# budzianowski/VAEB

Measured on AMD Instinct MI355X. Metric: SGVB training images/sec + ELBO at MNIST 784-500-20, batch 100, higher is better.
Workload: dtype f32; 1 GPU; MNIST 784-500-20 Bernoulli decoder, LB estimator, L=1, Adagrad lr 0.01; global_batch=100, batch_per_gpu=100, parallelism=dp1

## Files before the change

include/vaeb_diag.h:

```cpp
#ifndef VAEB_DIAG_H
#define VAEB_DIAG_H

#include "vaeb_hip.h"

#ifdef __cplusplus
extern "C" {
#endif

int vaeb_profile_steps(vaeb_ctx* ctx, int32_t n_steps, float* out_ms_per_kernel,
                       int32_t* out_kernel_ids, int32_t max_kernels, int32_t* out_n_kernels);
int vaeb_kernel_name(int32_t kernel_id, char* out, int32_t cap);

enum vaeb_graph_mode { VAEB_GRAPH_OFF = 0, VAEB_GRAPH_NOT_CAPTURED = 1, VAEB_GRAPH_REPLAY = 2,
                       VAEB_GRAPH_EAGER_FALLBACK = 3 };
int vaeb_graph_status(vaeb_ctx* ctx, int32_t* mode, char* msg, int32_t cap);
int vaeb_time_update_many(vaeb_ctx* ctx, const int32_t* batch_indices, int32_t n, float* out_gpu_ms,
                          double* out_enqueue_ms);
int vaeb_busy(vaeb_ctx* ctx, int32_t us);
int vaeb_comm_info(vaeb_ctx* ctx, int32_t* rccl_version, int32_t* dp_overlap, int32_t* world);
int vaeb_dp_plan(const vaeb_config* cfg, int32_t world, int32_t rank, int32_t sharded, int32_t bucket,
                 int64_t* out_P, int64_t* runs, int32_t* out_nrun, int64_t* own, int32_t* out_nown,
                 int32_t* out_book, int64_t* foreign, int32_t* out_nforeign);
int vaeb_dw2_plan(const vaeb_config* cfg, int32_t* out_width, int32_t* out_paired, int32_t* out_workers,
                  int32_t* out_free_cus, int32_t* out_split, int32_t* ranges, int32_t cap);
int vaeb_dp_rank_update(vaeb_ctx* ctx, int32_t world, int32_t rank, int32_t bucket, const float* grad_sum,
                        int64_t n_grad, const float* theta_gathered, int32_t finish);
int vaeb_get_shadow(vaeb_ctx* ctx, uint16_t* out, int64_t n);
int vaeb_debug_timeline(vaeb_ctx* ctx, int32_t batch_index, uint64_t* out, int64_t cap,
                        int32_t* out_launches);

int vaeb_test_gemm_bf16(vaeb_ctx* ctx, int32_t a_kouter, int32_t b_kouter, int32_t M, int32_t N, int32_t K,
                        const float* A, const float* B, float* C, int32_t ksplit);
int vaeb_bench_gemm_bf16(vaeb_ctx* ctx, int32_t a_kouter, int32_t b_kouter, int32_t M, int32_t N, int32_t K,
                         int32_t tile_n, int32_t reps, float* out_ms);

#ifdef __cplusplus
}
#endif
#endif
```

vaeb_amd/_lib.py:

```python
from __future__ import annotations

import ctypes
import os

import numpy as np

HERE = os.path.dirname(os.path.abspath(__file__))
LIB_PATH = os.path.join(HERE, "libvaeb_hip.so")
if os.environ.get("VAEB_LIB_VARIANT"):
    LIB_PATH = os.path.join(HERE, f"libvaeb_hip_{os.environ['VAEB_LIB_VARIANT']}.so")

DEC_BERNOULLI, DEC_GAUSSIAN = 0, 1
EST_LB, EST_LA, EST_FV, EST_FVS = 0, 1, 2, 3
OBJ_SUM_PRIOR, OBJ_MEAN_MAP = 0, 1
EPS_PHILOX, EPS_HOST = 0, 1
DTYPE_F32, DTYPE_BF16, DTYPE_F16 = 0, 1, 2

EXPORTS = [
    "vaeb_last_error", "vaeb_version", "vaeb_create", "vaeb_destroy", "vaeb_num_params",
    "vaeb_set_data", "vaeb_set_params", "vaeb_get_params", "vaeb_set_adagrad_state",
    "vaeb_get_adagrad_state", "vaeb_set_fv_state", "vaeb_get_fv_state", "vaeb_set_eps_mode",
    "vaeb_push_eps", "vaeb_set_step", "vaeb_get_step", "vaeb_update", "vaeb_update_async", "vaeb_update_many",
    "vaeb_epoch_elbo", "vaeb_synchronize", "vaeb_validate", "vaeb_reconstruct", "vaeb_reconstruct_sampled",
    "vaeb_reconstruct_full", "vaeb_decode", "vaeb_encode", "vaeb_marginal_ll", "vaeb_marginal_ll_resident",
    "vaeb_comm_unique_id", "vaeb_comm_init", "vaeb_comm_count", "vaeb_set_valid_data", "vaeb_validate_resident",
    "vaeb_checkpoint_save", "vaeb_checkpoint_load", "vaeb_get_grads", "vaeb_get_activation", "vaeb_push_fv_noise",
    "vaeb_ae_create", "vaeb_ae_destroy", "vaeb_ae_num_params", "vaeb_ae_set_data", "vaeb_ae_set_params",
    "vaeb_ae_get_params", "vaeb_ae_set_adagrad_state", "vaeb_ae_get_adagrad_state", "vaeb_ae_train",
    "vaeb_ae_train_many", "vaeb_ae_reconstruct", "vaeb_ae_encode", "vaeb_ae_decode",
]
DIAG_EXPORTS = ["vaeb_profile_steps", "vaeb_kernel_name", "vaeb_debug_timeline", "vaeb_test_gemm_bf16",
                "vaeb_bench_gemm_bf16", "vaeb_graph_status", "vaeb_comm_info", "vaeb_time_update_many", "vaeb_busy",
                "vaeb_dp_plan", "vaeb_dp_rank_update", "vaeb_get_shadow", "vaeb_dw2_plan"]
GRAPH_MODES = {0: "off", 1: "not_captured", 2: "replay", 3: "eager_fallback"}
AE_MAX_LAYERS = 8
AE_BINARY, AE_CONT = 0, 1
ACT = {"tanh": 0, "sigmoid": 1, "relu": 2}


class VaebConfig(ctypes.Structure):
    _fields_ = [
        ("D", ctypes.c_int32), ("H", ctypes.c_int32), ("Z", ctypes.c_int32), ("B", ctypes.c_int32),
        ("B_global", ctypes.c_int32), ("row_offset", ctypes.c_int32), ("L", ctypes.c_int32),
        ("decoder", ctypes.c_int32), ("estimator", ctypes.c_int32), ("objective", ctypes.c_int32),
        ("lr", ctypes.c_float), ("adagrad_eps", ctypes.c_float), ("device", ctypes.c_int32),
        ("max_eval_rows", ctypes.c_int32), ("use_graph", ctypes.c_int32), ("keep_grads", ctypes.c_int32),
        ("dtype", ctypes.c_int32), ("reserved", ctypes.c_int32 * 5),
    ]


class AEConfigC(ctypes.Structure):
    _fields_ = [
        ("Dobs", ctypes.c_int32), ("n_enc", ctypes.c_int32), ("Denc", ctypes.c_int32 * 8),
        ("Dz", ctypes.c_int32), ("n_dec", ctypes.c_int32), ("Ddec", ctypes.c_int32 * 8),
        ("otype", ctypes.c_int32), ("act", ctypes.c_int32), ("s2", ctypes.c_float), ("eta", ctypes.c_float),
        ("max_batch", ctypes.c_int32), ("device", ctypes.c_int32), ("reserved", ctypes.c_int32 * 4),
    ]


class VaebError(RuntimeError):
    pass


_lib = None

_F = ctypes.POINTER(ctypes.c_float)
_I64 = ctypes.c_int64
_P = ctypes.c_void_p


def load():
    global _lib
    if _lib is not None:
        return _lib
    if not os.path.exists(LIB_PATH):
        raise VaebError(f"{LIB_PATH} not found: build it with `python -c 'import __graft_entry__ as g; g.build()'`")
    if not os.environ.get("VAEB_LIB_VARIANT"):
        from ._buildinfo import check_stamp
        why = check_stamp(LIB_PATH)
        if why:
            raise VaebError(f"stale {LIB_PATH}: {why}; rebuild with `python -c 'import __graft_entry__ as g; g.build()'`")
    lib = ctypes.CDLL(LIB_PATH)
    sig = {
        "vaeb_last_error": ([], ctypes.c_char_p),
        "vaeb_version": ([ctypes.POINTER(ctypes.c_int32)] * 2, ctypes.c_int),
        "vaeb_create": ([ctypes.POINTER(VaebConfig), ctypes.POINTER(_P)], ctypes.c_int),
        "vaeb_destroy": ([_P], ctypes.c_int),
        "vaeb_num_params": ([_P, ctypes.POINTER(_I64)], ctypes.c_int),
        "vaeb_set_data": ([_P, _F, _I64], ctypes.c_int),
        "vaeb_set_params": ([_P, _F, _I64], ctypes.c_int),
        "vaeb_get_params": ([_P, _F, _I64], ctypes.c_int),
        "vaeb_set_adagrad_state": ([_P, _F, _I64], ctypes.c_int),
        "vaeb_get_adagrad_state": ([_P, _F, _I64], ctypes.c_int),
        "vaeb_set_fv_state": ([_P, _F, _F, _F, _F, _I64], ctypes.c_int),
        "vaeb_get_fv_state": ([_P, _F, _F, _F, _F, _I64], ctypes.c_int),
        "vaeb_set_eps_mode": ([_P, ctypes.c_int32, ctypes.c_uint64], ctypes.c_int),
        "vaeb_push_eps": ([_P, _F, _I64, ctypes.c_int32], ctypes.c_int),
        "vaeb_set_step": ([_P, _I64], ctypes.c_int),
        "vaeb_get_step": ([_P, ctypes.POINTER(_I64)], ctypes.c_int),
        "vaeb_comm_count": ([_P, ctypes.POINTER(ctypes.c_int32)], ctypes.c_int),
        "vaeb_set_valid_data": ([_P, _F, _I64], ctypes.c_int),
        "vaeb_validate_resident": ([_P, ctypes.POINTER(ctypes.c_double)], ctypes.c_int),
        "vaeb_checkpoint_save": ([_P, ctypes.c_char_p], ctypes.c_int),
        "vaeb_checkpoint_load": ([_P, ctypes.c_char_p], ctypes.c_int),
        "vaeb_update": ([_P, ctypes.c_int32, _F], ctypes.c_int),
        "vaeb_update_async": ([_P, ctypes.c_int32], ctypes.c_int),
        "vaeb_update_many": ([_P, ctypes.POINTER(ctypes.c_int32), ctypes.c_int32], ctypes.c_int),
        "vaeb_epoch_elbo": ([_P, ctypes.POINTER(ctypes.c_double), ctypes.POINTER(_I64)], ctypes.c_int),
        "vaeb_synchronize": ([_P], ctypes.c_int),
        "vaeb_validate": ([_P, _F, _I64, ctypes.POINTER(ctypes.c_double)], ctypes.c_int),
        "vaeb_reconstruct": ([_P, _F, _I64, _F], ctypes.c_int),
        "vaeb_reconstruct_sampled": ([_P, _F, _I64, ctypes.c_int32, _F], ctypes.c_int),
        "vaeb_reconstruct_full": ([_P, _F, _I64, ctypes.c_int32, _F, _F], ctypes.c_int),
        "vaeb_decode": ([_P, _F, _I64, _F, _F], ctypes.c_int),
        "vaeb_encode": ([_P, _F, _I64, _F, _F], ctypes.c_int),
        "vaeb_marginal_ll": ([_P, _F, _I64, ctypes.c_int32, ctypes.POINTER(ctypes.c_double), _F], ctypes.c_int),
        "vaeb_marginal_ll_resident": ([_P, ctypes.c_int32, ctypes.POINTER(ctypes.c_double)], ctypes.c_int),
        "vaeb_comm_unique_id": ([ctypes.POINTER(ctypes.c_uint8)], ctypes.c_int),
        "vaeb_comm_init": ([_P, ctypes.POINTER(ctypes.c_uint8), ctypes.c_int32, ctypes.c_int32], ctypes.c_int),
        "vaeb_get_grads": ([_P, _F, _I64], ctypes.c_int),
        "vaeb_get_activation": ([_P, ctypes.c_char_p, _F, _I64], ctypes.c_int),
        "vaeb_profile_steps": ([_P, ctypes.c_int32, _F, ctypes.POINTER(ctypes.c_int32), ctypes.c_int32,
                                ctypes.POINTER(ctypes.c_int32)], ctypes.c_int),
        "vaeb_kernel_name": ([ctypes.c_int32, ctypes.c_char_p, ctypes.c_int32], ctypes.c_int),
        "vaeb_graph_status": ([_P, ctypes.POINTER(ctypes.c_int32), ctypes.c_char_p, ctypes.c_int32], ctypes.c_int),
        "vaeb_comm_info": ([_P] + [ctypes.POINTER(ctypes.c_int32)] * 3, ctypes.c_int),
        "vaeb_busy": ([_P, ctypes.c_int32], ctypes.c_int),
        "vaeb_dp_plan": ([ctypes.POINTER(VaebConfig)] + [ctypes.c_int32] * 4 +
                         [ctypes.POINTER(_I64), ctypes.POINTER(_I64), ctypes.POINTER(ctypes.c_int32),
                          ctypes.POINTER(_I64), ctypes.POINTER(ctypes.c_int32), ctypes.POINTER(ctypes.c_int32),
                          ctypes.POINTER(_I64), ctypes.POINTER(ctypes.c_int32)], ctypes.c_int),
        "vaeb_dp_rank_update": ([_P] + [ctypes.c_int32] * 3 + [_F, _I64, _F, ctypes.c_int32], ctypes.c_int),
        "vaeb_dw2_plan": ([ctypes.POINTER(VaebConfig)] + [ctypes.POINTER(ctypes.c_int32)] * 6 + [ctypes.c_int32],
                          ctypes.c_int),
        "vaeb_get_shadow": ([_P, ctypes.POINTER(ctypes.c_uint16), _I64], ctypes.c_int),
        "vaeb_time_update_many": ([_P, ctypes.POINTER(ctypes.c_int32), ctypes.c_int32, _F,
                                   ctypes.POINTER(ctypes.c_double)], ctypes.c_int),
        "vaeb_debug_timeline": ([_P, ctypes.c_int32, ctypes.POINTER(ctypes.c_uint64), _I64,
                                 ctypes.POINTER(ctypes.c_int32)], ctypes.c_int),
        "vaeb_test_gemm_bf16": ([_P] + [ctypes.c_int32] * 5 + [_F, _F, _F, ctypes.c_int32], ctypes.c_int),
        "vaeb_bench_gemm_bf16": ([_P] + [ctypes.c_int32] * 7 + [_F], ctypes.c_int),
        "vaeb_push_fv_noise": ([_P, _F, _I64], ctypes.c_int),
        "vaeb_ae_create": ([ctypes.POINTER(AEConfigC), ctypes.POINTER(_P)], ctypes.c_int),
        "vaeb_ae_destroy": ([_P], ctypes.c_int),
        "vaeb_ae_num_params": ([_P, ctypes.POINTER(_I64)], ctypes.c_int),
        "vaeb_ae_set_data": ([_P, _F, _I64], ctypes.c_int),
        "vaeb_ae_set_params": ([_P, _F, _I64], ctypes.c_int),
        "vaeb_ae_get_params": ([_P, _F, _I64], ctypes.c_int),
        "vaeb_ae_set_adagrad_state": ([_P, _F, _I64], ctypes.c_int),
        "vaeb_ae_get_adagrad_state": ([_P, _F, _I64], ctypes.c_int),
        "vaeb_ae_train": ([_P, ctypes.POINTER(ctypes.c_int32), ctypes.c_int32, _F], ctypes.c_int),
        "vaeb_ae_train_many": ([_P, ctypes.POINTER(ctypes.c_int32), ctypes.c_int32, ctypes.c_int32, _F], ctypes.c_int),
        "vaeb_ae_reconstruct": ([_P, _F, _I64, _F], ctypes.c_int),
        "vaeb_ae_encode": ([_P, _F, _I64, _F], ctypes.c_int),
        "vaeb_ae_decode": ([_P, _F, _I64, _F], ctypes.c_int),
    }
    for name, (args, res) in sig.items():
        fn = getattr(lib, name)
        fn.argtypes = args
        fn.restype = res
    _lib = lib
    return lib


def check(rc):
    if rc != 0:
        msg = _lib.vaeb_last_error().decode(errors="replace") if _lib is not None else "?"
        raise VaebError(f"libvaeb_hip error {rc}: {msg}")


def dp_plan(D, H, Z, world, rank, bucket=2, sharded=True, decoder=DEC_BERNOULLI):
    lib = load()
    cfg = VaebConfig()
    cfg.D, cfg.H, cfg.Z, cfg.B, cfg.L = D, H, Z, 1, 1
    cfg.decoder = decoder
    P = _I64()
    runs = (_I64 * 9)()
    own = (_I64 * 12)()
    foreign = (_I64 * 12)()
    nrun, nown, book, nfor = (ctypes.c_int32() for _ in range(4))
    check(lib.vaeb_dp_plan(ctypes.byref(cfg), world, rank, int(bool(sharded)), bucket, ctypes.byref(P), runs,
                           ctypes.byref(nrun), own, ctypes.byref(nown), ctypes.byref(book), foreign,
                           ctypes.byref(nfor)))
    return {"P": P.value,
            "runs": [(runs[3 * j], runs[3 * j + 1], runs[3 * j + 2]) for j in range(nrun.value)],
            "own": [(own[2 * k], own[2 * k + 1]) for k in range(nown.value)],
            "book": bool(book.value),
            "foreign": [(foreign[2 * k], foreign[2 * k + 1]) for k in range(nfor.value)]}


def dw2_plan(D, H, Z, B, decoder=DEC_BERNOULLI):
    lib = load()
    cfg = VaebConfig()
    cfg.D, cfg.H, cfg.Z, cfg.B, cfg.B_global, cfg.L = D, H, Z, B, B, 1
    cfg.decoder = decoder
    width, paired, workers, free, split = (ctypes.c_int32() for _ in range(5))
    check(lib.vaeb_dw2_plan(ctypes.byref(cfg), ctypes.byref(width), ctypes.byref(paired), ctypes.byref(workers),
                            ctypes.byref(free), ctypes.byref(split), None, 0))
    r = (ctypes.c_int32 * (4 * workers.value))()
    check(lib.vaeb_dw2_plan(ctypes.byref(cfg), None, None, None, None, None, r, workers.value))
    return {"width": width.value, "paired": bool(paired.value), "workers": workers.value, "free_cus": free.value,
            "split": split.value, "ranges": [tuple(r[4 * k:4 * k + 4]) for k in range(workers.value)]}


def fptr(a: np.ndarray):
    assert a.dtype == np.float32 and a.flags["C_CONTIGUOUS"]
    return a.ctypes.data_as(_F)


class Context:

    def __init__(self, D, H, Z, B, L=1, decoder=DEC_BERNOULLI, estimator=EST_LB, objective=OBJ_SUM_PRIOR,
                 lr=0.01, adagrad_eps=1e-6, device=0, B_global=None, row_offset=0, max_eval_rows=10000,
                 use_graph=True, keep_grads=False, dtype=DTYPE_F32):
        self.lib = load()
        cfg = VaebConfig()
        cfg.D, cfg.H, cfg.Z, cfg.B, cfg.L = D, H, Z, B, L
        cfg.B_global = B if B_global is None else B_global
        cfg.row_offset = row_offset
        cfg.decoder, cfg.estimator, cfg.objective = decoder, estimator, objective
        cfg.lr, cfg.adagrad_eps = lr, adagrad_eps
        cfg.device, cfg.max_eval_rows = device, max_eval_rows
        cfg.use_graph, cfg.keep_grads = int(bool(use_graph)), int(bool(keep_grads))
        cfg.dtype = int(dtype)
        self.cfg = cfg
        self.h = _P()
        check(self.lib.vaeb_create(ctypes.byref(cfg), ctypes.byref(self.h)))
        n = _I64()
        check(self.lib.vaeb_num_params(self.h, ctypes.byref(n)))
        self.P = n.value

    def close(self):
        if getattr(self, "h", None) is not None and self.h.value:
            self.lib.vaeb_destroy(self.h)
            self.h = _P()

    def __del__(self):
        try:
            self.close()
        except Exception:
            pass

    def set_data(self, x):
        x = np.ascontiguousarray(x, np.float32)
        check(self.lib.vaeb_set_data(self.h, fptr(x), x.shape[0]))

    def set_params(self, flat):
        flat = np.ascontiguousarray(flat, np.float32)
        check(self.lib.vaeb_set_params(self.h, fptr(flat), flat.size))

    def get_params(self):
        out = np.empty(self.P, np.float32)
        check(self.lib.vaeb_get_params(self.h, fptr(out), out.size))
        return out

    def set_adagrad_state(self, flat):
        flat = np.ascontiguousarray(flat, np.float32)
# ... 312 lines not shown
```

vaeb_amd/csrc/latent.hpp:

```cpp
#pragma once
#include <type_traits>
#include "fused.hpp"
#include "kernels_aux.hpp"

namespace vaeb {

typedef unsigned int u32x4 __attribute__((ext_vector_type(4)));

DEV void st4_sc1(rsrc_t b, uint32_t off, f32x4 v) {
    __builtin_amdgcn_raw_buffer_store_b128(__builtin_bit_cast(u32x4, v), b, off, 0, 16);
}
DEV f32x4 ld4_sc1(rsrc_t b, uint32_t off) {
    return __builtin_bit_cast(f32x4, __builtin_amdgcn_raw_buffer_load_b128(b, off, 0, 16));
}

template <int NSW = 1>
DEV bool arrive_last(int* cnt, int target, int* sflag) {
    if constexpr (NSW > 1) {
        if ((int)threadIdx.x < 64 * NSW) asm volatile("s_waitcnt vmcnt(0)" ::: "memory");
        __syncthreads();
    }
    if (threadIdx.x < 64) {
        if constexpr (NSW == 1) asm volatile("s_waitcnt vmcnt(0)" ::: "memory");
        if (threadIdx.x == 0) {
// ... 400 lines not shown
    constexpr bool v1 = V1;
    typename PD::PreRow pre{};
    f32x4 acc[NT];
#pragma unroll
    for (int w = 0; w < NT; ++w) acc[w] = zero4();
    f32x4 w1v[ZS], b1v[4];
    float w2b[4][4][NT];
    auto load_block = [&](int kb) {
#pragma unroll
        for (int t = 0; t < ZS; ++t) {
            const int c = 4 * t + q, k = kb + 4 * li;
            w1v[t] = kc4(bw1, H, c, k, Z, H, v1);
        }
#pragma unroll
        for (int r = 0; r < 4; ++r) b1v[r] = kc4(bb1, 0, 0, kb + 16 * q + 4 * r, 1, H, v1);
#pragma unroll
        for (int u = 0; u < 4; ++u)
#pragma unroll
            for (int r = 0; r < 4; ++r)
#pragma unroll
                for (int w = 0; w < NT; ++w) {
                    const int k = kb + 16 * q + 4 * r + u;
                    w2b[u][r][w] = p.b1(n0 + 16 * (w / NB) + li, k, w % NB);
                }
    };
    constexpr int kSlabPer = 6;
    f32x4 sv0[ZM == 2 ? kSlabPer : 1];
    const int nctS = (H + 31) >> 5, nf4S = 8 * Z;
    const int npS = 512 / nf4S;
    const int fS = (int)threadIdx.x % nf4S, partS = (int)threadIdx.x / nf4S;
    const rsrc_t bsl = mkbuf(a.slab_ml, ZM == 2 ? (int64_t)(a.Mbp >> 4) * nctS * nf4S * 16 : 0);
    const int64_t firstS = (int64_t)((m0 % a.Mbp) >> 4) * nctS * nf4S + fS;
    if constexpr (ZM == 2) {
#pragma unroll
        for (int u = 0; u < kSlabPer; ++u) {
            const int ct = partS + u * npS;
            sv0[u] = bld4(bsl, (partS < npS && ct < nctS) ? (uint32_t)((firstS + (int64_t)ct * nf4S) * 16) : kOOB);
        }
    }
    load_block(64 * wave);
    float zb[ZS];
    if constexpr (!AT) {
        const rsrc_t bz = mkbuf(a.z, (int64_t)a.Me * Z * 4);
#pragma unroll
        for (int t = 0; t < ZS; ++t) zb[t] = bld(bz, (4 * t + q < Z) ? (uint32_t)((m0 + li) * Z + 4 * t + q) * 4u : kOOB);
    } else {
        __shared__ float zs[16][33];
        __shared__ float gs[16][33];
        __shared__ float msum[ZM >= 2 ? 64 : 1][17];
        __shared__ f32x4 spart[ZM == 2 ? 512 : 1];
        const int per = 16 * Z;
        const int l = m0 / a.Mbp;
        const int i0 = m0 - l * a.Mbp;
        float b4p = 0.f, b5p = 0.f, epre = 0.f;
        int64_t stp = 0, grow0p = 0;
        if constexpr (ZM >= 2) {
            if ((int)threadIdx.x < per) {
                const int ml = threadIdx.x / Z, j = threadIdx.x - ml * Z;
                b4p = a.b4[j];
                b5p = a.b5[j];
                if (a.eps_mode == 1 && i0 + ml < a.Mb) epre = a.eps_in[((int64_t)l * a.eps_in_ld + i0 + ml) * Z + j];
            }
            stp = a.step ? *a.step : 0;
            grow0p = (a.order ? (int64_t)ld_launch_const(a.cursor + kCtlNext) * a.row_base_mul : 0) + a.row_base_add;
        }
        if constexpr (ZM == 2) {
            const int nct = nctS, nf4 = nf4S, np = npS, f = fS, part = partS;
            const int64_t first = firstS;
            f32x4 sum = zero4();
#pragma unroll
            for (int u = 0; u < kSlabPer; ++u) sum += sv0[u];
            for (int c0 = part + kSlabPer * np; c0 < nct; c0 += kSlabPer * np) {
                f32x4 v[kSlabPer];
#pragma unroll
                for (int u = 0; u < kSlabPer; ++u) {
                    const int ct = c0 + u * np;
                    v[u] = bld4(bsl, (part < np && ct < nct) ? (uint32_t)((first + (int64_t)ct * nf4) * 16) : kOOB);
                }
#pragma unroll
                for (int u = 0; u < kSlabPer; ++u) sum += v[u];
            }
            spart[threadIdx.x] = sum;
            __syncthreads();
            if ((int)threadIdx.x < nf4) {
                f32x4 t = spart[threadIdx.x];
                for (int pp = 1; pp < np; ++pp) t += spart[pp * nf4 + threadIdx.x];
                const int c = threadIdx.x >> 2, mq = threadIdx.x & 3;
#pragma unroll
                for (int k = 0; k < 4; ++k) msum[c][4 * mq + k] = t[k];
            }
            __syncthreads();
            VAEB_STAMP(a, 6);
        }
        if ((int)threadIdx.x < per) {
            const int ml = threadIdx.x / Z, j = threadIdx.x - ml * Z;
            const int i = i0 + ml;
            const bool rv = i < a.Mb;
            float mu, lv, e;
            if constexpr (ZM >= 2) {
                mu = rv ? msum[j][ml] + b4p : 0.f;
                lv = rv ? msum[Z + j][ml] + b5p : 0.f;
                e = 0.f;
                if (rv) {
                    if (a.eps_mode == 0) e = philox_normal(a.seed, (uint32_t)(grow0p + i), (uint32_t)(l * Z + j), philox_c23(stp, a.domain));
                    else if (a.eps_mode == 1) e = epre;
                }
                if (col0) {
                    a.eps[((int64_t)l * a.Mbp + i) * Z + j] = e;
                    if (l == 0) {
                        a.mu[(int64_t)i * Z + j] = mu;
                        a.lv[(int64_t)i * Z + j] = lv;
                    }
                }
            } else {
                mu = a.mu[(int64_t)i * Z + j];
                lv = a.lv[(int64_t)i * Z + j];
                e = a.eps[((int64_t)l * a.Mbp + i) * Z + j];
            }
            const float z = rv ? mu + fexp(0.5f * lv) * e : 0.f;
            zs[ml][j] = z;
            if (col0) {
                a.z[((int64_t)l * a.Mbp + i) * Z + j] = z;
                const float elv = fexp(lv);
                float g;
                if (a.est == EST_LA) {
                    const float d = z - mu;
                    g = (-0.5f * z * z) - (-0.5f * lv - 0.5f * d * d / elv);
                } else {
                    g = 0.5f * (1.f + lv - mu * mu - elv);
                }
                gs[ml][j] = rv ? g : 0.f;
            }
        }
        __syncthreads();
        VAEB_STAMP(a, 7);
#pragma unroll
        for (int t = 0; t < ZS; ++t) zb[t] = (4 * t + q < Z) ? zs[li][4 * t + q] : 0.f;
        if (col0 && threadIdx.x < 16 && (a.est == EST_LA || l == 0)) {
            float f = 0.f;
            for (int j = 0; j < Z; ++j) f += gs[threadIdx.x][j];
            const int i = i0 + threadIdx.x;
            float* dst = a.est == EST_LA ? a.la_part + ((int64_t)l * a.Mbp + i) * a.nctZ : a.kl_part + (int64_t)i * a.nctZ;
            for (int n = 0; n < a.nctZ; ++n) dst[n] = n == 0 ? f : 0.f;
        }
    }
    for (int kb = 64 * wave; kb < H; kb += 64 * 8) {
        if (kb != 64 * wave) load_block(kb);
        if (kb == 64 * wave && wave < 4 * CT) {
            p.x = x_rows(a);
            pre = p.prefetch_row(m0, n0 + 16 * (wave >> 2), wave & 3);
        }
        f32x4 hv[4];
#pragma unroll
        for (int u = 0; u < 4; ++u) {
            f32x4 t = zero4();
#pragma unroll
            for (int st = 0; st < ZS; ++st) t = __builtin_amdgcn_mfma_f32_16x16x4f32(w1v[st][u], zb[st], t, 0, 0, 0);
// ... 64 lines not shown
```

vaeb_amd/csrc/vaeb_hip.hip:

```cpp
#include <hip/hip_runtime.h>
#include <rccl/rccl.h>

#include <algorithm>
#include <chrono>
#include <cmath>
#include <cstdarg>
#include <cstdlib>
#include <cstdio>
#include <cstring>
#include <string>
#include <vector>
#include <type_traits>

#include "../../include/vaeb_diag.h"
#include "hfuse.hpp"
#include "latent.hpp"
#include "latent_bwd.hpp"
#include "iwae.hpp"
#include "h16_engines.hpp"
#include "ae_mlp.hpp"

using namespace vaeb;

namespace {

thread_local std::string g_err;

int fail(int code, const char* fmt, ...) {
    char buf[512];
    va_list ap;
    va_start(ap, fmt);
    vsnprintf(buf, sizeof(buf), fmt, ap);
    va_end(ap);
    g_err = buf;
    return code;
}

#define HIP_TRY(expr)                                                                      \
    do {                                                                                   \
        hipError_t e_ = (expr);                                                            \
        if (e_ != hipSuccess) {                                                            \
            (void)hipGetLastError();  \
            return fail(VAEB_ERR_HIP, "%s failed: %s (%s:%d)", #expr, hipGetErrorString(e_), \
                        __FILE__, __LINE__);                                               \
        }                                                                                  \
    } while (0)

#define CHECK_LAUNCH()                                                                     \
    do {                                                                                   \
        hipError_t e_ = hipGetLastError();                                                 \
        if (e_ != hipSuccess)                                                              \
            return fail(VAEB_ERR_HIP, "kernel launch failed: %s (%s:%d)",                  \
                        hipGetErrorString(e_), __FILE__, __LINE__);                        \
    } while (0)

inline int r16(int x) { return (x + 15) & ~15; }
inline int cdiv(int64_t a, int64_t b) { return (int)((a + b - 1) / b); }

template <class T>
int dalloc(T** p, size_t n) {
    if (n == 0) n = 1;
    hipError_t e = hipMalloc((void**)p, n * sizeof(T));
    if (e != hipSuccess) return fail(VAEB_ERR_NOMEM, "hipMalloc(%zu) failed: %s", n * sizeof(T), hipGetErrorString(e));
    e = hipMemset(*p, 0, n * sizeof(T));
    if (e == hipSuccess) e = hipStreamSynchronize(nullptr);
    if (e != hipSuccess) return fail(VAEB_ERR_HIP, "zero fill of %zu bytes: %s", n * sizeof(T), hipGetErrorString(e));
    return 0;
}

constexpr int kFvParts = 1024;
constexpr int kGraphSteps = 32;
constexpr int kMaxProfKernels = 24;
constexpr int kDbgWG = 1024;

const char* kKernelNames[] = {"p1_enc", "p2_heads", "p3_dechid", "p4_decout", "p5_dhd_w2", "p6_dz",
                              "p7_dh", "p8_wgrad_w3w45", "allreduce", "adagrad", "fv_update", "elbo",
                              "p23_heads_dechid", "p67_dz_dh_w1", "p8_wgrad_w2", "p8_wgrad_w1",
                              "p1_enc_latent", "p4_decout_z",
                              "bf_enc", "bf_heads", "bf_latent", "bf_dechid", "bf_decout", "bf_dhd", "bf_dW26",
                              "bf_dz", "bf_dW1", "bf_dW1_opt", "bf_latent_bwd", "bf_dh", "bf_dW45", "bf_dW45_opt",
                              "bf_dW3", "bf_bias_elbo", "bf_adagrad_dp",
                              "unused35", "unused36", "fvs_sample", "fvs_update",
                              "p5_dhd_dz_w2", "p8_wgrad_w3w45w1",
                              "bf_dhd_dW26",
                              "p1_enc_latent_w2", "p5_dhd_dz"};

}

struct vaeb_ctx {
    vaeb_config c{};
    hipStream_t s = nullptr;
    int64_t P = 0;
    int nparams = 0;
    int64_t off[12] = {};
    float* theta2[2] = {nullptr, nullptr};
    int par = 0;
    float *acc = nullptr, *grad = nullptr;
    float *fvmu = nullptr, *fvsg = nullptr, *fvam = nullptr, *fvas = nullptr, *fv_part = nullptr;
    float* fvzeta = nullptr;
    float* data = nullptr;
    int64_t nrows = 0;
    float* xeval = nullptr;
    float* xval = nullptr;
    int64_t nval = 0;
    int* ictl = nullptr;
    int64_t* step = nullptr;
    float* elbo_out = nullptr;
    double* epoch = nullptr;
    uint64_t* blk = nullptr;
    double* eval_acc = nullptr;
    int eps_mode = VAEB_EPS_PHILOX;
    uint64_t seed = 10;
    float* eps_in = nullptr;
    int64_t eps_in_cap = 0, eps_rows = 0;
    int cap = 0;
    float *h = nullptr, *mu = nullptr, *lv = nullptr, *eps = nullptr, *z = nullptr, *hd = nullptr,
          *y = nullptr, *dA2 = nullptr, *dA6 = nullptr, *dA1 = nullptr, *dZ = nullptr,
          *dMuLv = nullptr, *dA3 = nullptr, *kl_part = nullptr, *lp_part = nullptr;
    float* yacc = nullptr;
    float* iw = nullptr;
    float *slab_ml = nullptr, *slab_dz = nullptr;
    int *cnt_ml = nullptr, *cnt_dz = nullptr;
    uint64_t *acc_ml = nullptr, *acc_dz = nullptr;
    int* h_ctl = nullptr;
    float* h_elbo = nullptr;
    double* h_d2 = nullptr;
    float* h_out = nullptr;
    bool async_pending = false;
    hipEvent_t ctl_ev = nullptr;
    hipGraphExec_t gN[2][kGraphSteps + 1] = {};
    bool graph_failed = false;
    std::string graph_err;
    ncclComm_t comm = nullptr;
    int rank = 0, world = 1;
    hipStream_t s3 = nullptr;
    hipEvent_t fk_ev[4] = {};
    int bf_thin = 3;
    bool bf_fork = true;
    int bf_dzfuse = 1;
    int bf_dtt = 1;
    hipStream_t s2 = nullptr;
    hipEvent_t dp_ev[3] = {};
    bool dp_overlap = false;
    bool dp_shard = false;
    bool fold_bwd = true;
    bool bwd_defer = true;
    bool dw2_defer = true;
    bool dw2_paired = false;
    int* w2pend = nullptr;
    bool w2_dirty = false;
    bool w2_graph = false;
    int atomic_ho = 1;
    int enc_red = -1;
    bool order_pending = false;
    OrderArg order_pend;
    hipEvent_t pev[kMaxProfKernels + 1] = {};
    int prof_n = 0, prof_reps = 1;
    std::vector<int> prof_ids;
    uint64_t* dbg = nullptr;
    int dbg_slot = 0;
    h16c::BfState bf;
};

namespace {

bool gaussian(const vaeb_ctx* c) { return c->c.decoder == VAEB_DEC_GAUSSIAN; }

void set_arena_layout(vaeb_ctx* c) {
    const int64_t D = c->c.D, H = c->c.H, Z = c->c.Z;
    std::vector<int64_t> sz = {D * H, H * Z, H * Z, Z * H, H * D};
    if (gaussian(c)) sz.push_back(H * D);
    sz.insert(sz.end(), {H, Z, Z, H, D});
    if (gaussian(c)) sz.push_back(D);
    c->nparams = (int)sz.size();
    int64_t o = 0;
    for (int i = 0; i < c->nparams; ++i) { c->off[i] = o; o += sz[i]; }
    c->P = o;
}

uint64_t* next_dbg(vaeb_ctx* c) { return c->dbg ? c->dbg + (size_t)(c->dbg_slot++) * kDbgWG * 8 : nullptr; }

int order_hook(vaeb_ctx* c);

// ... 819 lines not shown
        WGroup g12[3] = {
            make_group(c, nullptr, a.D, a.Mb, 1, a.D, c->dA3, a.H, a.H, nullptr, 0, 0, a.Mbp, 0, bo + 0, -1, -1),
            make_group(c, c->h, a.H, a.Mbp, 0, a.H, c->dMuLv, 2 * a.Z, a.Z, c->dMuLv + a.Z, 2 * a.Z, a.Z, a.Mbp, 1,
                       bo + 1, 2, bo + 2),
            make_group(c, c->z, a.Z, a.Me, 0, a.Z, c->dA1, a.H, a.H, nullptr, 0, 0, a.Me, 3, bo + 3, -1, -1)};
        ElboArgs e1 = e;
        if (dp || fvs) { e1.dp_slot = c->grad + c->P; e1.elbo_out = nullptr; e1.cursor = nullptr; e1.step = nullptr; }
        a.dbg = next_dbg(c);
        if (fold) {
            Da3Src d3{c->dMuLv, a.W4, a.W5, c->h, c->dA3, a.Z, a.H, a.Mb, a.Mbp, LatRed{}};
            if (ho_dz(c) == 2) {
                LatRed& r = d3.red;
                r.slab = c->slab_dz; r.mu = c->mu; r.lv = c->lv; r.eps = c->eps; r.z = c->z;
                r.dZ = c->dZ; r.dml = c->dMuLv; r.cnt = c->cnt_dz; r.guard = c->blk + kBlkFxErr;
                r.ngrp = cdiv(a.Z, 8); r.zg = cdiv(a.Z, r.ngrp);
                if (a.Z % 4 == 0) { r.zg = (r.zg + 3) & ~3; r.ngrp = cdiv(a.Z, r.zg); }
                r.nred = (a.Mbp / 16) * r.ngrp;
                r.nctH = cdiv(a.H, 16); r.L = a.L; r.est = a.est; r.Mb = a.Mb; r.Mbp = a.Mbp; r.Z = a.Z; r.sc = a.sc;
            }
            pr.mark(40);
            REP(pr) if (int rc = launch_wgrad(c, s, g12, 3, opt, &e1, a, &d3)) return rc;
        } else {
            pr.mark(7);
            REP(pr) if (int rc = launch_wgrad(c, s, g12, 2, opt, &e1, a)) return rc;
        }
    }
    if (fvs) {
        pr.mark(38);
        REP(pr) hipLaunchKernelGGL(fvs_update_kernel, dim3(kFvParts), dim3(256), 0, s, c->fvmu, c->fvsg, c->fvam,
                                   c->fvas, (const float*)c->grad, c->P, (float)g.B, g.lr, g.adagrad_eps, c->seed,
                                   (const int64_t*)c->step, zin, c->fv_part, zin ? nullptr : c->theta2[par]);
        CHECK_LAUNCH();
        pr.mark(11);
        e.fv_part = c->fv_part; e.n_fv = kFvParts;
        e.data_mul = (double)g.B;
        e.est = VAEB_EST_FV;
        hipLaunchKernelGGL(elbo_kernel, dim3(1), dim3(256), 0, s, e);
        CHECK_LAUNCH();
    }
    if (dp) if (int rc = dp_bucket_b(c, pr, 9, dopt.theta_out, dp_opt, no_fix)) return rc;
    pr.mark(-1);
    c->prof_n = pr.k;
    return 0;
}

bool flips(const vaeb_ctx* c) { return c->c.estimator != VAEB_EST_FV && c->c.estimator != VAEB_EST_FVS; }

void free_graphs(vaeb_ctx* c) {
    for (auto& fam : c->gN)
        for (auto& gn : fam) {
            if (gn) hipGraphExecDestroy(gn);
            gn = nullptr;
        }
    c->w2_graph = false;
}

int capture(vaeb_ctx* c, int nsteps, int par, hipGraphExec_t* out) {
    hipGraph_t gr = nullptr;
    HIP_TRY(hipStreamBeginCapture(c->s, hipStreamCaptureModeThreadLocal));
    int rc = 0;
    const bool dirty0 = c->w2_dirty;
    c->w2_dirty = false;
    for (int i = 0; i < nsteps && rc == 0; ++i) {
        rc = enqueue_train_step(c, par, false, i == 0);
        if (flips(c)) par ^= 1;
    }
    if (c->w2_dirty) c->w2_graph = true;
    c->w2_dirty = dirty0;
    hipError_t e = hipStreamEndCapture(c->s, &gr);
    if (rc) { if (gr) hipGraphDestroy(gr); return rc; }
    if (e != hipSuccess) return fail(VAEB_ERR_HIP, "hipStreamEndCapture: %s", hipGetErrorString(e));
    e = hipGraphInstantiate(out, gr, nullptr, nullptr, 0);
    hipGraphDestroy(gr);
    if (e != hipSuccess) return fail(VAEB_ERR_HIP, "hipGraphInstantiate: %s", hipGetErrorString(e));
    if (hipGraphUpload(*out, c->s) != hipSuccess) (void)hipGetLastError();
    return 0;
}

int step_eager(vaeb_ctx* c, int direct = -1) {
    if (int rc = enqueue_train_step(c, c->par, false, true, direct)) return rc;
    if (flips(c)) c->par ^= 1;
    return 0;
}

int run_steps(vaeb_ctx* c, int n) {
    if (c->c.use_graph && !c->graph_failed) {
        if (!c->gN[0][1]) {
            int rc = 0;
            for (int p = 0; p < (flips(c) ? 2 : 1); ++p)
                for (int m = 1; m <= kGraphSteps && rc == 0; ++m) rc = capture(c, m, p, &c->gN[p][m]);
            if (rc) {
                c->graph_failed = true;
                c->graph_err = g_err;
                free_graphs(c);
                (void)hipGetLastError();
                if (c->comm && c->world > 1)
                    return fail(VAEB_ERR_HIP, "graph capture of the data-parallel step failed at world %d: %s",
                                c->world, c->graph_err.c_str());
            }
        }
        if (!c->graph_failed) {
            for (int i = 0; i < n;) {
                const int m = std::min(kGraphSteps, n - i), p = flips(c) ? c->par : 0;
                HIP_TRY(hipGraphLaunch(c->gN[p][m], c->s));
                if (flips(c)) c->par = p ^ (m & 1);
                i += m;
            }
            if (n > 0 && c->w2_graph) c->w2_dirty = true;
            return 0;
        }
    }
    for (int i = 0; i < n; ++i)
        if (int rc = step_eager(c)) return rc;
    return 0;
}

int order_hook(vaeb_ctx* c) {
    if (!c->order_pending) return 0;
    c->order_pending = false;
    hipLaunchKernelGGL(set_order_kernel, dim3(1), dim3(256), 0, c->s, c->ictl, c->order_pend);
    CHECK_LAUNCH();
    return 0;
}

int upload_order(vaeb_ctx* c, const int32_t* idx, int n) {
    if (n <= kArgOrder) {
        OrderArg u;
        u.n = n;
        memcpy(u.v, idx, sizeof(int) * (size_t)n);
        hipLaunchKernelGGL(set_order_kernel, dim3(1), dim3(256), 0, c->s, c->ictl, u);
        CHECK_LAUNCH();
        return 0;
    }
    HIP_TRY(hipEventSynchronize(c->ctl_ev));
    c->h_ctl[0] = 0;
    c->h_ctl[1] = 0;
    c->h_ctl[kCtlNext] = n > 0 ? idx[0] : 0;
    memcpy(c->h_ctl + kCtlOrder, idx, sizeof(int) * (size_t)n);
    HIP_TRY(hipMemcpyAsync(c->ictl, c->h_ctl, sizeof(int) * (size_t)(n + kCtlOrder), hipMemcpyHostToDevice, c->s));
    HIP_TRY(hipEventRecord(c->ctl_ev, c->s));
    return 0;
}

int check_batches(vaeb_ctx* c, const int32_t* idx, int n) {
    if (!c->data) return fail(VAEB_ERR_STATE, "vaeb_set_data has not been called");
    const int64_t nb = c->nrows / c->c.B_global;
    for (int i = 0; i < n; ++i)
        if (idx[i] < 0 || idx[i] >= nb)
            return fail(VAEB_ERR_ARG, "batch index %d out of range [0, %lld)", idx[i], (long long)nb);
    return 0;
}


}

extern "C" {

const char* vaeb_last_error(void) { return g_err.c_str(); }

int vaeb_version(int32_t* major, int32_t* minor) {
    if (major) *major = 0;
    if (minor) *minor = 2;
    return 0;
}

int vaeb_create(const vaeb_config* cfg, vaeb_ctx** out) {
    if (!cfg || !out) return fail(VAEB_ERR_ARG, "null argument");
    const vaeb_config& g = *cfg;
    if (g.D <= 0 || g.H <= 0 || g.Z <= 0 || g.B <= 0 || g.L <= 0)
        return fail(VAEB_ERR_ARG, "dimensions must be positive (D=%d H=%d Z=%d B=%d L=%d)", g.D, g.H, g.Z, g.B, g.L);
    if (g.decoder < 0 || g.decoder > 1 || g.estimator < 0 || g.estimator > 3 || g.objective < 0 || g.objective > 1)
        return fail(VAEB_ERR_ARG, "bad decoder/estimator/objective enum");
    const bool fvx = g.estimator == VAEB_EST_FV || g.estimator == VAEB_EST_FVS;
    if (fvx && g.L != 1)
        return fail(VAEB_ERR_ARG, "the full-variational estimators support L == 1 only (VAEB.py:361)");
    if (g.dtype != VAEB_DTYPE_F32 && g.dtype != VAEB_DTYPE_BF16 && g.dtype != VAEB_DTYPE_F16)
        return fail(VAEB_ERR_ARG, "bad dtype %d", g.dtype);
    if (g.dtype == VAEB_DTYPE_BF16 || g.dtype == VAEB_DTYPE_F16) {
        if (g.D % 8 || g.H % 8 || g.Z % 8)
            return fail(VAEB_ERR_ARG, "bf16 engine: D, H, Z must be multiples of 8 (got %d, %d, %d)", g.D, g.H, g.Z);
        if (g.decoder == VAEB_DEC_GAUSSIAN && g.D % 32)
            return fail(VAEB_ERR_ARG, "bf16 engine: the Gaussian decoder needs D %% 32 == 0 (got %d)", g.D);
        if (fvx) return fail(VAEB_ERR_ARG, "bf16 engine: the FV estimators run on the fp32 path");
        if (g.estimator == VAEB_EST_LA && g.L > 8) return fail(VAEB_ERR_ARG, "bf16 engine: LA supports L <= 8");
    }
    auto* c = new vaeb_ctx();
    c->c = g;
    if (c->c.B_global <= 0) c->c.B_global = g.B;
    if (c->c.adagrad_eps <= 0.f) c->c.adagrad_eps = 1e-6f;
    if (c->c.max_eval_rows <= 0) c->c.max_eval_rows = 10000;
    hipError_t e = hipSetDevice(g.device);
    if (e != hipSuccess) { delete c; return fail(VAEB_ERR_HIP, "hipSetDevice(%d): %s", g.device, hipGetErrorString(e)); }
    e = hipStreamCreateWithFlags(&c->s, hipStreamNonBlocking);
    if (const char* fb = getenv("VAEB_FOLD_BWD")) c->fold_bwd = atoi(fb) != 0;
    if (const char* bd = getenv("VAEB_BWD_DEFER")) c->bwd_defer = atoi(bd) != 0;
    if (const char* wd = getenv("VAEB_DW2_DEFER")) c->dw2_defer = atoi(wd) != 0;
    if (const char* wp = getenv("VAEB_DW2_PAIRED")) c->dw2_paired = atoi(wp) != 0;
    if (const char* ah = getenv("VAEB_ATOMIC_HO")) c->atomic_ho = atoi(ah) != 0 ? 1 : 0;
    if (const char* er = getenv("VAEB_ENC_RED")) c->enc_red = atoi(er) != 0 ? 1 : 0;
    if (const char* bk = getenv("VAEB_BF_FORK")) c->bf_fork = atoi(bk) != 0;
    if (const char* tt = getenv("VAEB_BF_DTT")) c->bf_dtt = atoi(tt) != 0;
    if (const char* zf = getenv("VAEB_BF_DZFUSE")) c->bf_dzfuse = atoi(zf) != 0;
    if (const char* bt = getenv("VAEB_BF_THIN")) c->bf_thin = atoi(bt) & 3;
    {
        const char* g8 = getenv("VAEB_BF_GEMM8");
        g_gemm8 = g8 ? (int)strtol(g8, nullptr, 0) : 11;
    }
    if (e != hipSuccess) { delete c; return fail(VAEB_ERR_HIP, "stream/event create: %s", hipGetErrorString(e)); }
    const int64_t D = g.D, H = g.H, Z = g.Z;
    set_arena_layout(c);
    c->cap = std::max(r16(g.B), r16(c->c.max_eval_rows));
    const int64_t R = c->cap, RL = (int64_t)c->cap * g.L;
    int rc = 0;
    rc = rc ? rc : dalloc(&c->theta2[0], c->P);
    rc = rc ? rc : dalloc(&c->theta2[1], c->P);
    rc = rc ? rc : dalloc(&c->acc, c->P);
    rc = rc ? rc : dalloc(&c->grad, c->P + 1);
    if (g.estimator == VAEB_EST_FV || g.estimator == VAEB_EST_FVS) {
        rc = rc ? rc : dalloc(&c->fvmu, c->P);
        rc = rc ? rc : dalloc(&c->fvsg, c->P);
        rc = rc ? rc : dalloc(&c->fvam, c->P);
        rc = rc ? rc : dalloc(&c->fvas, c->P);
    }
    rc = rc ? rc : dalloc(&c->fv_part, kFvParts);
    rc = rc ? rc : dalloc(&c->xeval, (size_t)R * D);
    rc = rc ? rc : dalloc(&c->ictl, kCtlOrder + kOrderCap);
    rc = rc ? rc : dalloc(&c->step, 1);
    rc = rc ? rc : dalloc(&c->eval_acc, 2);
    rc = rc ? rc : dalloc(&c->h, (size_t)R * H);
    rc = rc ? rc : dalloc(&c->mu, (size_t)R * Z);
    rc = rc ? rc : dalloc(&c->lv, (size_t)R * Z);
    rc = rc ? rc : dalloc(&c->eps, (size_t)RL * Z);
    rc = rc ? rc : dalloc(&c->z, (size_t)RL * Z);
    rc = rc ? rc : dalloc(&c->hd, (size_t)RL * H);
    rc = rc ? rc : dalloc(&c->y, (size_t)RL * D);
    rc = rc ? rc : dalloc(&c->dA2, (size_t)RL * D * (gaussian(c) ? 2 : 1));
    if (!rc && gaussian(c)) c->dA6 = c->dA2 + (size_t)RL * D;
    rc = rc ? rc : dalloc(&c->dA1, (size_t)RL * H);
    rc = rc ? rc : dalloc(&c->dZ, (size_t)RL * Z);
    rc = rc ? rc : dalloc(&c->dMuLv, (size_t)R * 2 * Z);
    rc = rc ? rc : dalloc(&c->dA3, (size_t)R * H);
    rc = rc ? rc : dalloc(&c->kl_part, (size_t)RL * cdiv(Z, 16));
    rc = rc ? rc : dalloc(&c->lp_part, (size_t)RL * cdiv(D, 16));
    {
        const int64_t Bp = r16(g.B), nctH = cdiv(H, 16);
        rc = rc ? rc : dalloc(&c->slab_ml, (size_t)(Bp * nctH * 64));
        rc = rc ? rc : dalloc(&c->slab_dz, (size_t)(g.L * Bp * nctH * 32));
        rc = rc ? rc : dalloc(&c->cnt_ml, (size_t)(Bp / 16));
        rc = rc ? rc : dalloc(&c->cnt_dz, (size_t)std::max<int64_t>(Bp / 16, kLatCnt * kLatCntStride));
        rc = rc ? rc : dalloc(&c->w2pend, 1);
        const size_t nacc = (size_t)(Bp * 2 * Z * kFxStride);
        rc = rc ? rc : dalloc(&c->blk, kBlkAcc + 2 * nacc);
        if (!rc) {
            c->epoch = reinterpret_cast<double*>(c->blk);
            c->elbo_out = reinterpret_cast<float*>(c->blk + kBlkElbo);
            c->acc_ml = c->blk + kBlkAcc;
// ... 888 lines not shown
    HIP_TRY(hipMemcpy(out, d, m * sizeof(uint64_t), hipMemcpyDeviceToHost));
    hipFree(d);
    if (out_launches) *out_launches = launches;
    return 0;
}

int vaeb_test_gemm_bf16(vaeb_ctx* c, int32_t ako, int32_t bko, int32_t M, int32_t N, int32_t K, const float* A,
                        const float* B, float* C, int32_t ksplit) {
    if (!c) return fail(VAEB_ERR_ARG, "null ctx");
    return is_f16(c) ? eng_hf::h16_test_gemm(c, ako, bko, M, N, K, A, B, C, ksplit)
                     : eng_bf::h16_test_gemm(c, ako, bko, M, N, K, A, B, C, ksplit);
}

int vaeb_bench_gemm_bf16(vaeb_ctx* c, int32_t ako, int32_t bko, int32_t M, int32_t N, int32_t K, int32_t bn,
                         int32_t reps, float* out_ms) {
    if (!c) return fail(VAEB_ERR_ARG, "null ctx");
    return is_f16(c) ? eng_hf::h16_bench_gemm(c, ako, bko, M, N, K, bn, reps, out_ms)
                     : eng_bf::h16_bench_gemm(c, ako, bko, M, N, K, bn, reps, out_ms);
}

int vaeb_time_update_many(vaeb_ctx* c, const int32_t* idx, int32_t n, float* out_gpu_ms, double* out_enqueue_ms) {
    if (!c || !out_gpu_ms) return fail(VAEB_ERR_ARG, "null argument");
    hipEvent_t e0 = nullptr, e1 = nullptr;
    HIP_TRY(hipEventCreate(&e0));
    HIP_TRY(hipEventCreate(&e1));
    HIP_TRY(hipStreamSynchronize(c->s));
    HIP_TRY(hipEventRecord(e0, c->s));
    const auto t0 = std::chrono::steady_clock::now();
    int rc = vaeb_update_many(c, idx, n);
    const auto t1 = std::chrono::steady_clock::now();
    if (rc == 0) {
        hipEventRecord(e1, c->s);
        hipEventSynchronize(e1);
        hipEventElapsedTime(out_gpu_ms, e0, e1);
        if (out_enqueue_ms) *out_enqueue_ms = std::chrono::duration<double, std::milli>(t1 - t0).count();
    }
    hipEventDestroy(e0);
    hipEventDestroy(e1);
    return rc;
}

int vaeb_busy(vaeb_ctx* c, int32_t us) {
    if (!c || us <= 0) return fail(VAEB_ERR_ARG, "bad arguments");
    hipLaunchKernelGGL(busy_kernel, dim3(2048), dim3(256), 0, c->s, (uint64_t)us * 100, c->fv_part);
    CHECK_LAUNCH();
    return 0;
}

int vaeb_graph_status(vaeb_ctx* c, int32_t* mode, char* msg, int32_t cap) {
    if (!c || !mode) return fail(VAEB_ERR_ARG, "null argument");
    if (!c->c.use_graph) *mode = VAEB_GRAPH_OFF;
    else if (c->graph_failed) *mode = VAEB_GRAPH_EAGER_FALLBACK;
    else *mode = c->gN[0][1] ? VAEB_GRAPH_REPLAY : VAEB_GRAPH_NOT_CAPTURED;
    if (msg && cap > 0) snprintf(msg, (size_t)cap, "%s", c->graph_failed ? c->graph_err.c_str() : "");
    return 0;
}

int vaeb_comm_info(vaeb_ctx* c, int32_t* rccl_version, int32_t* dp_overlap, int32_t* world) {
    if (!c) return fail(VAEB_ERR_ARG, "null ctx");
    if (rccl_version) {
        int v = 0;
        ncclResult_t r = ncclGetVersion(&v);
        if (r != ncclSuccess) return fail(VAEB_ERR_COMM, "ncclGetVersion: %s", ncclGetErrorString(r));
        *rccl_version = v;
    }
    if (dp_overlap) *dp_overlap = c->comm ? (c->dp_overlap ? 1 : 0) : -1;
    if (world) *world = c->comm ? c->world : 1;
    return 0;
}

int vaeb_dp_plan(const vaeb_config* cfg, int32_t world, int32_t rank, int32_t sharded, int32_t bucket,
                 int64_t* out_P, int64_t* runs, int32_t* out_nrun, int64_t* own, int32_t* out_nown, int32_t* out_book,
                 int64_t* foreign, int32_t* out_nforeign) {
    if (!cfg || world <= 0 || rank < 0 || rank >= world || bucket < 0 || bucket > 2)
        return fail(VAEB_ERR_ARG, "bad plan arguments");
    if (cfg->D <= 0 || cfg->H <= 0 || cfg->Z <= 0) return fail(VAEB_ERR_ARG, "dimensions must be positive");
    vaeb_ctx c;
    c.c = *cfg;
    set_arena_layout(&c);
    c.world = world;
    c.rank = rank;
    c.dp_shard = sharded != 0;
    const DpBucket bk = bucket == 0 ? dp_bucket_a_runs(&c) : bucket == 1 ? dp_bucket_b_runs(&c) : dp_bucket_all_runs(&c);
    if (out_P) *out_P = c.P;
    if (runs)
        for (int j = 0; j < bk.nrun; ++j) {
            runs[3 * j] = bk.lo[j];
            runs[3 * j + 1] = bk.n[j];
            runs[3 * j + 2] = dp_shard_len(&c, bk.n[j]);
        }
    if (out_nrun) *out_nrun = bk.nrun;
    auto put = [](const DpRange& r, int64_t* dst, int32_t* cnt) {
        int k = 0;
        while (k < kDpRuns && r.n[k]) {
            if (dst) { dst[2 * k] = r.lo[k]; dst[2 * k + 1] = r.n[k]; }
            ++k;
        }
        if (cnt) *cnt = k;
    };
    const DpRange o = dp_opt_range(&c, bk);
    put(o, own, out_nown);
    if (out_book) *out_book = o.book;
    put(dp_foreign_range(&c, bk), foreign, out_nforeign);
    return 0;
}

int vaeb_dw2_plan(const vaeb_config* cfg, int32_t* out_width, int32_t* out_paired, int32_t* out_workers,
// ... 115 lines not shown
```

Before: 2.998 million images/s.

## Add long 128-step graph replay and hoist Philox eps draw earlier

Captures an extra pair of HIP graphs covering 128 steps, one per parity arena, and replays them for long update_many calls instead of chunks of 32. This cuts the number of graph launches and the host-side launch overhead. Separately, the latent kernel now draws its Philox normal noise before the reduction rather than inside it, so the RNG cost can overlap with memory latency. The long graphs cost extra capture time and memory, and they fall back to short graphs if capture fails.

```diff
diff --git a/include/vaeb_diag.h b/include/vaeb_diag.h
--- a/include/vaeb_diag.h
+++ b/include/vaeb_diag.h
@@ -14,6 +14,8 @@
 enum vaeb_graph_mode { VAEB_GRAPH_OFF = 0, VAEB_GRAPH_NOT_CAPTURED = 1, VAEB_GRAPH_REPLAY = 2,
                        VAEB_GRAPH_EAGER_FALLBACK = 3 };
 int vaeb_graph_status(vaeb_ctx* ctx, int32_t* mode, char* msg, int32_t cap);
+int vaeb_graph_chunks(int32_t n, int32_t long_graph, int32_t par, int32_t flips, int32_t* out_len,
+                      int32_t* out_arena, int32_t cap, int32_t* out_n);
 int vaeb_time_update_many(vaeb_ctx* ctx, const int32_t* batch_indices, int32_t n, float* out_gpu_ms,
                           double* out_enqueue_ms);
 int vaeb_busy(vaeb_ctx* ctx, int32_t us);
diff --git a/vaeb_amd/_lib.py b/vaeb_amd/_lib.py
--- a/vaeb_amd/_lib.py
+++ b/vaeb_amd/_lib.py
@@ -31,7 +31,7 @@
 ]
 DIAG_EXPORTS = ["vaeb_profile_steps", "vaeb_kernel_name", "vaeb_debug_timeline", "vaeb_test_gemm_bf16",
                 "vaeb_bench_gemm_bf16", "vaeb_graph_status", "vaeb_comm_info", "vaeb_time_update_many", "vaeb_busy",
-                "vaeb_dp_plan", "vaeb_dp_rank_update", "vaeb_get_shadow", "vaeb_dw2_plan"]
+                "vaeb_dp_plan", "vaeb_dp_rank_update", "vaeb_get_shadow", "vaeb_dw2_plan", "vaeb_graph_chunks"]
 GRAPH_MODES = {0: "off", 1: "not_captured", 2: "replay", 3: "eager_fallback"}
 AE_MAX_LAYERS = 8
 AE_BINARY, AE_CONT = 0, 1
@@ -133,6 +133,8 @@
         "vaeb_dp_rank_update": ([_P] + [ctypes.c_int32] * 3 + [_F, _I64, _F, ctypes.c_int32], ctypes.c_int),
         "vaeb_dw2_plan": ([ctypes.POINTER(VaebConfig)] + [ctypes.POINTER(ctypes.c_int32)] * 6 + [ctypes.c_int32],
                           ctypes.c_int),
+        "vaeb_graph_chunks": ([ctypes.c_int32] * 4 + [ctypes.POINTER(ctypes.c_int32)] * 2 +
+                              [ctypes.c_int32, ctypes.POINTER(ctypes.c_int32)], ctypes.c_int),
         "vaeb_get_shadow": ([_P, ctypes.POINTER(ctypes.c_uint16), _I64], ctypes.c_int),
         "vaeb_time_update_many": ([_P, ctypes.POINTER(ctypes.c_int32), ctypes.c_int32, _F,
                                    ctypes.POINTER(ctypes.c_double)], ctypes.c_int),
@@ -203,6 +205,15 @@
             "split": split.value, "ranges": [tuple(r[4 * k:4 * k + 4]) for k in range(workers.value)]}
 
 
+def graph_chunks(n, long_graph=128, par=0, flips=True):
+    lib = load()
+    cnt = ctypes.c_int32()
+    check(lib.vaeb_graph_chunks(n, long_graph, par, int(bool(flips)), None, None, 0, ctypes.byref(cnt)))
+    ln, ar = (ctypes.c_int32 * max(1, cnt.value))(), (ctypes.c_int32 * max(1, cnt.value))()
+    check(lib.vaeb_graph_chunks(n, long_graph, par, int(bool(flips)), ln, ar, cnt.value, ctypes.byref(cnt)))
+    return [(ln[k], ar[k]) for k in range(cnt.value)]
+
+
 def fptr(a: np.ndarray):
     assert a.dtype == np.float32 and a.flags["C_CONTIGUOUS"]
     return a.ctypes.data_as(_F)
diff --git a/vaeb_amd/csrc/latent.hpp b/vaeb_amd/csrc/latent.hpp
--- a/vaeb_amd/csrc/latent.hpp
+++ b/vaeb_amd/csrc/latent.hpp
@@ -476,8 +476,7 @@
         const int per = 16 * Z;
         const int l = m0 / a.Mbp;
         const int i0 = m0 - l * a.Mbp;
-        float b4p = 0.f, b5p = 0.f, epre = 0.f;
-        int64_t stp = 0, grow0p = 0;
+        float b4p = 0.f, b5p = 0.f, epre = 0.f, edraw = 0.f;
         if constexpr (ZM >= 2) {
             if ((int)threadIdx.x < per) {
                 const int ml = threadIdx.x / Z, j = threadIdx.x - ml * Z;
@@ -485,8 +484,13 @@
                 b5p = a.b5[j];
                 if (a.eps_mode == 1 && i0 + ml < a.Mb) epre = a.eps_in[((int64_t)l * a.eps_in_ld + i0 + ml) * Z + j];
             }
-            stp = a.step ? *a.step : 0;
-            grow0p = (a.order ? (int64_t)ld_launch_const(a.cursor + kCtlNext) * a.row_base_mul : 0) + a.row_base_add;
+            const int64_t stp = a.step ? *a.step : 0;
+            const int64_t grow0p = (a.order ? (int64_t)ld_launch_const(a.cursor + kCtlNext) * a.row_base_mul : 0) + a.row_base_add;
+            if ((int)threadIdx.x < per && a.eps_mode == 0) {
+                const int ml = threadIdx.x / Z, j = threadIdx.x - ml * Z;
+                if (i0 + ml < a.Mb)
+                    edraw = philox_normal(a.seed, (uint32_t)(grow0p + i0 + ml), (uint32_t)(l * Z + j), philox_c23(stp, a.domain));
+            }
         }
         if constexpr (ZM == 2) {
             const int nct = nctS, nf4 = nf4S, np = npS, f = fS, part = partS;
@@ -526,7 +530,7 @@
                 lv = rv ? msum[Z + j][ml] + b5p : 0.f;
                 e = 0.f;
                 if (rv) {
-                    if (a.eps_mode == 0) e = philox_normal(a.seed, (uint32_t)(grow0p + i), (uint32_t)(l * Z + j), philox_c23(stp, a.domain));
+                    if (a.eps_mode == 0) e = edraw;
                     else if (a.eps_mode == 1) e = epre;
                 }
                 if (col0) {
diff --git a/vaeb_amd/csrc/vaeb_hip.hip b/vaeb_amd/csrc/vaeb_hip.hip
--- a/vaeb_amd/csrc/vaeb_hip.hip
+++ b/vaeb_amd/csrc/vaeb_hip.hip
@@ -70,6 +70,7 @@
 
 constexpr int kFvParts = 1024;
 constexpr int kGraphSteps = 32;
+constexpr int kLongSteps = 128, kLongStepsMax = 1024;
 constexpr int kMaxProfKernels = 24;
 constexpr int kDbgWG = 1024;
 
@@ -129,6 +130,9 @@
     bool async_pending = false;
     hipEvent_t ctl_ev = nullptr;
     hipGraphExec_t gN[2][kGraphSteps + 1] = {};
+    hipGraphExec_t gL[2] = {};
+    int long_steps = kLongSteps;
+    bool long_failed = false;
     bool graph_failed = false;
     std::string graph_err;
     ncclComm_t comm = nullptr;
@@ -1054,10 +1058,34 @@
             if (gn) hipGraphExecDestroy(gn);
             gn = nullptr;
         }
+    for (auto& gl : c->gL) {
+        if (gl) hipGraphExecDestroy(gl);
+        gl = nullptr;
+    }
     c->w2_graph = false;
 }
 
+int long_graph_len(int v) {
+    v = std::min(v, kLongStepsMax) & ~1;
+    return v > kGraphSteps ? v : 0;
+}
+
+struct GraphChunk { int m, p; };
+std::vector<GraphChunk> graph_chunks(int n, int long_len, int par, bool flip) {
+    std::vector<GraphChunk> out;
+    int p = flip ? par : 0;
+    for (int i = 0; i < n;) {
+        const int left = n - i;
+        const int m = (long_len > 0 && left >= long_len) ? long_len : std::min(kGraphSteps, left);
+        out.push_back({m, p});
+        if (flip) p ^= m & 1;
+        i += m;
+    }
+    return out;
+}
+
 int capture(vaeb_ctx* c, int nsteps, int par, hipGraphExec_t* out) {
+    if (c->order_pending) return fail(VAEB_ERR_STATE, "graph capture with an order upload pending");
     hipGraph_t gr = nullptr;
     HIP_TRY(hipStreamBeginCapture(c->s, hipStreamCaptureModeThreadLocal));
     int rc = 0;
@@ -1101,12 +1129,25 @@
                                 c->world, c->graph_err.c_str());
             }
         }
+        const bool long_ok = !is_bf16(c) && !c->comm;
+        if (long_ok && !c->graph_failed && c->long_steps > 0 && n >= c->long_steps && !c->gL[0]) {
+            int rc = 0;
+            for (int p = 0; p < (flips(c) ? 2 : 1) && rc == 0; ++p) rc = capture(c, c->long_steps, p, &c->gL[p]);
+            if (rc) {
+                c->graph_err = g_err;
+                for (auto& gl : c->gL) {
+                    if (gl) hipGraphExecDestroy(gl);
+                    gl = nullptr;
+                }
+                c->long_steps = 0;
+                c->long_failed = true;
+                (void)hipGetLastError();
+            }
+        }
         if (!c->graph_failed) {
-            for (int i = 0; i < n;) {
-                const int m = std::min(kGraphSteps, n - i), p = flips(c) ? c->par : 0;
-                HIP_TRY(hipGraphLaunch(c->gN[p][m], c->s));
-                if (flips(c)) c->par = p ^ (m & 1);
-                i += m;
+            for (const GraphChunk& k : graph_chunks(n, c->gL[0] ? c->long_steps : 0, c->par, flips(c))) {
+                HIP_TRY(hipGraphLaunch(k.m > kGraphSteps ? c->gL[k.p] : c->gN[k.p][k.m], c->s));
+                if (flips(c)) c->par = k.p ^ (k.m & 1);
             }
             if (n > 0 && c->w2_graph) c->w2_dirty = true;
             return 0;
@@ -1204,6 +1245,7 @@
     if (const char* tt = getenv("VAEB_BF_DTT")) c->bf_dtt = atoi(tt) != 0;
     if (const char* zf = getenv("VAEB_BF_DZFUSE")) c->bf_dzfuse = atoi(zf) != 0;
     if (const char* bt = getenv("VAEB_BF_THIN")) c->bf_thin = atoi(bt) & 3;
+    if (const char* lg = getenv("VAEB_LONG_GRAPH")) c->long_steps = long_graph_len(atoi(lg));
     {
         const char* g8 = getenv("VAEB_BF_GEMM8");
         g_gemm8 = g8 ? (int)strtol(g8, nullptr, 0) : 11;
@@ -2198,7 +2240,19 @@
     if (!c->c.use_graph) *mode = VAEB_GRAPH_OFF;
     else if (c->graph_failed) *mode = VAEB_GRAPH_EAGER_FALLBACK;
     else *mode = c->gN[0][1] ? VAEB_GRAPH_REPLAY : VAEB_GRAPH_NOT_CAPTURED;
-    if (msg && cap > 0) snprintf(msg, (size_t)cap, "%s", c->graph_failed ? c->graph_err.c_str() : "");
+    if (msg && cap > 0) snprintf(msg, (size_t)cap, "%s", c->graph_failed || c->long_failed ? c->graph_err.c_str() : "");
+    return 0;
+}
+
+int vaeb_graph_chunks(int32_t n, int32_t long_graph, int32_t par, int32_t flips, int32_t* out_len,
+                      int32_t* out_arena, int32_t cap, int32_t* out_n) {
+    if (n < 0 || par < 0 || par > 1 || !out_n) return fail(VAEB_ERR_ARG, "bad chunk arguments");
+    const std::vector<GraphChunk> ch = graph_chunks(n, long_graph_len(long_graph), par, flips != 0);
+    for (int k = 0; k < (int)ch.size() && k < cap; ++k) {
+        if (out_len) out_len[k] = ch[k].m;
+        if (out_arena) out_arena[k] = ch[k].p;
+    }
+    *out_n = (int32_t)ch.size();
     return 0;
 }
 
```

Result: no change. 2.998 million images/s (median of 3 runs) (+0.0%).
